# submarine0418/underwater_image_enhancement

Measured on AMD Instinct MI355X. Metric: megapixels/sec enhanced, higher is better.
Workload: dtype f32/f64

## Files before the change

### underwater_image_enhancement_amd/csrc/k_fused.hip

```cpp
#include <cstdlib>

#include "common.h"
#include "devutil.h"
#include "restore.h"

namespace uwie {

namespace {


typedef float f32x2 __attribute__((ext_vector_type(2)));
#ifndef UWIE_CLAHE_PREFETCH
#define UWIE_CLAHE_PREFETCH 0
#endif
#ifndef UWIE_STRETCH_WAVES
#define UWIE_STRETCH_WAVES 5
#endif
#define UWIE_DESCALE(x, n) (((x) + (1 << ((n)-1))) >> (n))

template <bool LIN, bool COLLECT, int NW = 2, typename V = float>
__global__ void __launch_bounds__(256) k_restore_planar_hist(RestoreSrc S, int npx, V *__restrict__ planar,
                                                             uint32_t *__restrict__ ghist, LinState *__restrict__ lin,
                                                             V *__restrict__ lists, uint32_t cap)
{
// ... 357 lines not shown
    const RankWave X{img, tpl, ftab, a0, a1, a2, s_wlo, s_wspan, s_lo, s_hi, s_below, myq, wstg[wv],
                     &lin[3 * b].gcount[0], (uint32_t)(sizeof(LinState) / sizeof(uint32_t)),
                     lists + (size_t)(3 * b) * (kLinLists / kRankCapMul) * cap, cap, lane};

    const int step = gridDim.x * 1024, iters = (npx + step - 1) / step;
#define UWIE_RANK_LOAD4(p_, w_, tv_)                                                                                   \
    do {                                                                                                                \
        const u32_unaligned *q_ = reinterpret_cast<const u32_unaligned *>(img + (size_t)(p_) * 3);                      \
        (w_)[0] = q_[0]; (w_)[1] = q_[1]; (w_)[2] = q_[2];                                                              \
        const double2_a8 ta_ = *reinterpret_cast<const double2_a8 *>(tpl + (p_)),                                       \
                         tb_ = *reinterpret_cast<const double2_a8 *>(tpl + (p_) + 2);                                   \
        (tv_)[0] = ta_.x; (tv_)[1] = ta_.y; (tv_)[2] = tb_.x; (tv_)[3] = tb_.y;                                         \
    } while (0)
    uint32_t w_nx[3] = {0, 0, 0};
    double tv_nx[4] = {1.0, 1.0, 1.0, 1.0};
    bool have_nx = false;
    const int p_last = npx - 4;
    {
        const int p0 = (blockIdx.x * 256 + tid) * 4;
        have_nx = p0 + 4 <= npx;
        UWIE_RANK_LOAD4(min(p0, p_last), w_nx, tv_nx);
    }
    for (int it = 0; it < iters; ++it) {
        const int p = it * step + (blockIdx.x * 256 + tid) * 4;
        const bool have = have_nx;
        const uint32_t w0 = w_nx[0], w1 = w_nx[1], w2 = w_nx[2];
        const double tv[4] = {tv_nx[0], tv_nx[1], tv_nx[2], tv_nx[3]};
        {
            const int pn = p + step;
            have_nx = it + 1 < iters && pn + 4 <= npx;
            UWIE_RANK_LOAD4(min(pn, p_last), w_nx, tv_nx);
        }
        uint32_t fm = 0;
        seen += 4u * (uint32_t)__popcll(__ballot(have));
        if (have) {
            float y[4];
#pragma unroll
            for (int i = 0; i < 4; ++i) y[i] = __builtin_amdgcn_rcpf((float)tv[i]);
            const uint32_t ub[3][4] = {{w0 & 255, w0 >> 24, (w1 >> 16) & 255, (w2 >> 8) & 255},
                                       {(w0 >> 8) & 255, w1 & 255, w1 >> 24, (w2 >> 16) & 255},
                                       {(w0 >> 16) & 255, (w1 >> 8) & 255, w2 & 255, w2 >> 24}};
#pragma unroll
            for (int c = 0; c < 3; ++c) {
                const float ac = c == 0 ? a0 : c == 1 ? a1 : a2;
#pragma unroll
                for (int i = 0; i < 4; ++i) {
                    const float v = fmaf(ftab[c * 256 + (int)ub[c][i]], y[i], ac);
                    bool in = false;
#pragma unroll
                    for (int w = 0; w < NW; ++w) {
                        const bool ge = v >= elo[c * NW + w];
                        cnt[c * NW + w] += (uint32_t)__popcll(__ballot(ge));
                        in = in | (ge & (v <= ehi[c * NW + w]));
                    }
                    fm |= (uint32_t)in << (4 * c + i);
                }
                __builtin_amdgcn_sched_barrier(0);
            }
        }
        const bool ragged = !have && p < npx;
        const uint32_t nmine = (uint32_t)__popc(fm);
        if (__ballot(nmine != 0)) {
            uint32_t pre = 0, tot = 0;
#pragma unroll
            for (int bit = 0; bit < 4; ++bit) {
                const uint64_t mk = __ballot((nmine >> bit) & 1u);
                pre += (uint32_t)__popcll(mk & ((1ull << lane) - 1)) << bit;
                tot += (uint32_t)__popcll(mk) << bit;
            }
            uint32_t at = qn + pre;
            for (uint32_t f = fm; f; f &= f - 1, ++at) {
                const int k = __ffs(f) - 1;
                myq[at] = ((uint32_t)(p + (k & 3)) << 2) | (uint32_t)(k >> 2);
            }
            qn += tot;
            while (qn >= 64u) {
                qn -= 64u;
                rank_exact_batch(X, qn, 64u, true, sc);
            }
        }
        if (__ballot(ragged)) {
            const uint32_t n3 = ragged ? (uint32_t)(npx - p) * 3u : 0u;
            wave_lds_sync();
            if (ragged)
                for (uint32_t i = 0; i < n3; ++i) myq[qn + i] = ((uint32_t)(p + (int)(i / 3u)) << 2) | (i % 3u);
            const uint32_t m = (uint32_t)__builtin_amdgcn_readfirstlane((int)__shfl((int)n3, (int)__builtin_ctzll(__ballot(ragged))));
            rank_exact_batch(X, qn, m, false, sc);
        }
    }
    if (qn) rank_exact_batch(X, 0u, qn, true, sc);
#pragma unroll
    for (int j = 0; j < NS; ++j)
        if (sc[j]) rank_flush_stage(X, j, sc[j]);
#pragma unroll
    for (int j = 0; j < NS; ++j) {
        uint32_t k = cnt[j];
#pragma unroll
        for (int o = 32; o > 0; o >>= 1) k = max(k, (uint32_t)__shfl_xor((int)k, o));
        if (lane == 0 && seen != k) atomicAdd(&s_below[j], seen - k);
    }
    __syncthreads();
    if (tid < NS && s_below[tid]) atomicAdd(&lin[3 * b + tid / NW].below[tid % NW], s_below[tid]);
}

struct Stretch {
    StretchDiv d1[3], d2[3];
    float lo1[3], lo2[3];
    int two;
    __device__ __forceinline__ void load(const float *pct, int b, int stride, float eps, int two_)
    {
        two = two_;
#pragma unroll
        for (int c = 0; c < 3; ++c) {
            const float *p = pct + (size_t)(b * 3 + c) * stride;
            lo1[c] = p[0];
            d1[c].set((p[1] - p[0]) + eps);
            lo2[c] = two ? p[2] : 0.f;
            d2[c].set(two ? (p[3] - p[2]) + eps : 1.f);
        }
    }
    __device__ __forceinline__ float apply(float v, int c) const
    {
        v = clip01(d1[c].quot_unit(v - lo1[c]));
        if (two) v = clip01(d2[c].quot_unit(v - lo2[c]));
        return v;
    }
    __device__ __forceinline__ bool allfast() const { return !two && d1[0].fast && d1[1].fast && d1[2].fast; }
    __device__ __forceinline__ void codes4(const float (&v)[4], int c, uint32_t (&code)[4]) const
    {
        const float den = d1[c].den, y = d1[c].y, lo = lo1[c];
        const f32x2 nd = {-den, -den}, yy = {y, y};
#pragma unroll
        for (int h = 0; h < 2; ++h) {
            const f32x2 n = f32x2{v[2 * h], v[2 * h + 1]} - lo;
            f32x2 q = n * y;
            q = __builtin_elementwise_fma(__builtin_elementwise_fma(nd, q, n), yy, q);
            q = __builtin_elementwise_fma(__builtin_elementwise_fma(nd, q, n), yy, q);
            const f32x2 s = f32x2{clip01(q.x), clip01(q.y)} * 255.0f;
            code[2 * h] = (uint32_t)(int)s.x;
            code[2 * h + 1] = (uint32_t)(int)s.y;
        }
    }
    __device__ __forceinline__ float apply_exact(float v, int c) const
    {
        v = clip01(d1[c].quot(v - lo1[c]));
        if (two) v = clip01(d2[c].quot(v - lo2[c]));
        return v;
    }
};

struct ClaheGeom {
    int H, W, tx, ty, tw, th, clip;
    float lutScale;
};

template <int SRC, int BS = 256>
__global__ void __launch_bounds__(BS) __attribute__((amdgpu_waves_per_eu(BS == 256 ? UWIE_STRETCH_WAVES : 4, 8))) k_stretch_lab_lut(const LabTables *__restrict__ T, const float *__restrict__ planar,
                                                         RestoreSrc src, const float *__restrict__ pct, int pct_stride,
                                                         float eps, int two, const uint8_t *__restrict__ codes, ClaheGeom g,
                                                         uint8_t *__restrict__ lab, uint8_t *__restrict__ lut)
{
    __shared__ uint32_t h[4][256];
    __shared__ uint32_t wsum[4];
    __shared__ uint16_t s_gamma[256], s_cbrt[3072];
    __shared__ int s_fwd[9];
    const int tile = blockIdx.x, b = blockIdx.y, tid = threadIdx.x, w = (tid >> 6) & 3, w4 = w;
    for (int i = tid; i < 1024; i += BS) (&h[0][0])[i] = 0;
    for (int i = tid; i < 256; i += BS) s_gamma[i] = T->gamma[i];
    for (int i = tid; i < 3072; i += BS) s_cbrt[i] = T->cbrt[i];
    if (tid < 9) s_fwd[tid] = T->fwd[tid];
    __shared__ uint16_t s_gcode[SRC == 2 ? 768 : 1];
    Stretch S;
    if (SRC != 2) S.load(pct, b, pct_stride, eps, two);
    if (SRC == 2)
        for (int i = tid; i < 768; i += BS) s_gcode[i] = T->gamma[codes[(size_t)b * 768 + i]];
    __syncthreads();
    const int npx = g.H * g.W;
    const float *r0 = planar + (size_t)b * 3 * npx, *r1 = r0 + npx, *r2 = r1 + npx;
    const uint8_t *img8 = src.in + (size_t)b * npx * 3;
    __shared__ double dtab[SRC == 1 ? 768 : 1];
    auto pixels = [&](auto &R) {
    if (SRC == 1) {
        R.init(src, b, (size_t)npx, dtab);
        __syncthreads();
    }
    uint8_t *labimg = lab + (size_t)b * npx * 3;
    const int ty = tile / g.tx, txi = tile % g.tx;
    const int area = g.tw * g.th;
    constexpr int Lscale = (116 * 255 + 50) / 100;
    constexpr int Lshift = -((16 * 255 * (1 << 15) + 50) / 100);
    auto to_lab = [&](float v0, float v1, float v2, uint32_t &L, uint32_t &a, uint32_t &bb) {
        const int R = SRC == 2 ? s_gcode[(int)v0] : s_gamma[quant_u8(S.apply(v0, 0))];
        const int G = SRC == 2 ? s_gcode[256 + (int)v1] : s_gamma[quant_u8(S.apply(v1, 1))];
        const int B = SRC == 2 ? s_gcode[512 + (int)v2] : s_gamma[quant_u8(S.apply(v2, 2))];
        const int fX = s_cbrt[UWIE_DESCALE(R * s_fwd[0] + G * s_fwd[1] + B * s_fwd[2], 12)];
        const int fY = s_cbrt[UWIE_DESCALE(R * s_fwd[3] + G * s_fwd[4] + B * s_fwd[5], 12)];
        const int fZ = s_cbrt[UWIE_DESCALE(R * s_fwd[6] + G * s_fwd[7] + B * s_fwd[8], 12)];
        L = sat_u8(UWIE_DESCALE(Lscale * fY + Lshift, 15));
        a = sat_u8(UWIE_DESCALE(500 * (fX - fY) + 128 * (1 << 15), 15));
        bb = sat_u8(UWIE_DESCALE(200 * (fY - fZ) + 128 * (1 << 15), 15));
    };
    const int x_lo = txi * g.tw, x_hi = min(x_lo + g.tw, g.W), y_lo = ty * g.th, y_hi = min(y_lo + g.th, g.H);
    const int gpr = max((x_hi - x_lo + 3) / 4, 0), total = max(y_hi - y_lo, 0) * gpr;
    const uint32_t gmagic = (uint32_t)(((1ull << 32) + max(gpr, 1) - 1) / max(gpr, 1));
    const int f0 = T->fwd[0], f1 = T->fwd[1], f2 = T->fwd[2], f3 = T->fwd[3], f4 = T->fwd[4], f5 = T->fwd[5], f6 = T->fwd[6],
              f7 = T->fwd[7], f8 = T->fwd[8];
    auto lab_of = [&](uint32_t Rg, uint32_t Gg, uint32_t Bg, uint32_t &L, uint32_t &a, uint32_t &bb) {
        const uint32_t ix = (__umul24(Rg, f0) + __umul24(Gg, f1) + __umul24(Bg, f2) + 2048u) >> 12;
        const uint32_t iy = (__umul24(Rg, f3) + __umul24(Gg, f4) + __umul24(Bg, f5) + 2048u) >> 12;
        const uint32_t iz = (__umul24(Rg, f6) + __umul24(Gg, f7) + __umul24(Bg, f8) + 2048u) >> 12;
        const int fX = s_cbrt[ix], fY = s_cbrt[iy], fZ = s_cbrt[iz];
        auto sat15 = [](int x) { return (uint32_t)min(max(x, 0), (256 << 15) - 1) >> 15; };
        L = sat15(__mul24(Lscale, fY) + (Lshift + (1 << 14)));
        a = sat15(__mul24(500, fX - fY) + (128 * (1 << 15) + (1 << 14)));
        bb = sat15(__mul24(200, fY - fZ) + (128 * (1 << 15) + (1 << 14)));
    };
    const bool fastpath = SRC == 1 && S.allfast();
    auto group_at = [&](int gi, int &n, int &p) {
        const int row = gpr == 1 ? gi : (int)__umulhi((uint32_t)gi, gmagic), xg = gi - row * gpr;
        const int x0 = x_lo + 4 * xg;
        n = min(4, x_hi - x0);
        p = (y_lo + row) * g.W + x0;
    };
    uint32_t w_nx[3] = {0, 0, 0};
    double tv_nx[4] = {1.0, 1.0, 1.0, 1.0};
    bool have_nx = false;
    if (SRC == 1 && fastpath && tid < total) {
        int n0, p0;
        group_at(tid, n0, p0);
        have_nx = n0 == 4;
        if (have_nx) R.load_four(p0, w_nx, tv_nx);
    }
    for (int gi = tid; gi < total; gi += BS) {
        int n, p;
        group_at(gi, n, p);
        const bool have = have_nx;
        const uint32_t w[3] = {w_nx[0], w_nx[1], w_nx[2]};
        const double tv[4] = {tv_nx[0], tv_nx[1], tv_nx[2], tv_nx[3]};
        have_nx = false;
        if (SRC == 1 && fastpath && gi + BS < total) {
            int nn, pn;
            group_at(gi + BS, nn, pn);
            have_nx = nn == 4;
            if (have_nx) R.load_four(pn, w_nx, tv_nx);
        }
        if (SRC == 1 && have) {
            float v[3][4];
            R.four_raw(w, tv, v);
            uint32_t code[3][4];
#pragma unroll
            for (int c = 0; c < 3; ++c) {
                const float r[4] = {clip01(v[c][0]), clip01(v[c][1]), clip01(v[c][2]), clip01(v[c][3])};
                S.codes4(r, c, code[c]);
            }
            uint32_t L[4], a[4], bb[4];
#pragma unroll
            for (int i = 0; i < 4; ++i) lab_of(s_gamma[code[0][i]], s_gamma[code[1][i]], s_gamma[code[2][i]], L[i], a[i], bb[i]);
            uint32_t cl = L[0], cn = 1;
#pragma unroll
            for (int i = 1; i < 4; ++i) {
                if (L[i] == cl) {
                    ++cn;
                } else {
                    atomicAdd(&h[w4][cl], cn);
                    cl = L[i];
                    cn = 1;
                }
            }
            atomicAdd(&h[w4][cl], cn);
            u32_unaligned *wd = reinterpret_cast<u32_unaligned *>(labimg + (size_t)p * 3);
            wd[0] = L[0] | (a[0] << 8) | (bb[0] << 16) | (L[1] << 24);
            wd[1] = a[1] | (bb[1] << 8) | (L[2] << 16) | (a[2] << 24);
            wd[2] = bb[2] | (L[3] << 8) | (a[3] << 16) | (bb[3] << 24);
            continue;
        }
        float v0[4], v1[4], v2[4];
        if (SRC == 2) {
            const Px4 q = n == 4 ? load_px4_any(img8 + (size_t)p * 3) : load_px4(img8 + (size_t)p * 3, n, false);
#pragma unroll
            for (int i = 0; i < 4; ++i) {
                v0[i] = (float)q.r[i];
                v1[i] = (float)q.g[i];
                v2[i] = (float)q.b[i];
            }
        } else if (SRC == 1) {
            float r[3][4];
            R.four(p, n, r);
#pragma unroll
            for (int i = 0; i < 4; ++i) {
                v0[i] = r[0][i];
                v1[i] = r[1][i];
                v2[i] = r[2][i];
            }
        } else if (n == 4) {
            *reinterpret_cast<uint4 *>(v0) = *reinterpret_cast<const u128_unaligned *>(r0 + p);
            *reinterpret_cast<uint4 *>(v1) = *reinterpret_cast<const u128_unaligned *>(r1 + p);
            *reinterpret_cast<uint4 *>(v2) = *reinterpret_cast<const u128_unaligned *>(r2 + p);
        } else {
#pragma unroll
            for (int i = 0; i < 4; ++i) {
                v0[i] = i < n ? r0[p + i] : 0.f;
                v1[i] = i < n ? r1[p + i] : 0.f;
                v2[i] = i < n ? r2[p + i] : 0.f;
            }
        }
        uint32_t L[4], a[4], bb[4];
#pragma unroll
        for (int i = 0; i < 4; ++i) to_lab(v0[i], v1[i], v2[i], L[i], a[i], bb[i]);
        uint32_t cl = L[0], cn = 1;
#pragma unroll
        for (int i = 1; i < 4; ++i) {
            if (i >= n) break;
            if (L[i] == cl) {
                ++cn;
            } else {
                atomicAdd(&h[w4][cl], cn);
                cl = L[i];
                cn = 1;
            }
        }
        atomicAdd(&h[w4][cl], cn);
        uint8_t *o = labimg + (size_t)p * 3;
        if (n == 4) {
            u32_unaligned *wd = reinterpret_cast<u32_unaligned *>(o);
            wd[0] = L[0] | (a[0] << 8) | (bb[0] << 16) | (L[1] << 24);
            wd[1] = a[1] | (bb[1] << 8) | (L[2] << 16) | (a[2] << 24);
            wd[2] = bb[2] | (L[3] << 8) | (a[3] << 16) | (bb[3] << 24);
        } else {
            for (int i = 0; i < n; ++i) {
                o[3 * i] = (uint8_t)L[i];
                o[3 * i + 1] = (uint8_t)a[i];
                o[3 * i + 2] = (uint8_t)bb[i];
            }
        }
    }
    if (x_lo + g.tw > g.W || y_lo + g.th > g.H) {
        for (int i = tid; i < area; i += BS) {
            const int ey = ty * g.th + i / g.tw, ex = txi * g.tw + i % g.tw;
            if (ey < g.H && ex < g.W) continue;
            const int p = reflect101(ey, g.H) * g.W + reflect101(ex, g.W);
            uint32_t L, a, bb;
            float e0, e1, e2;
            if (SRC == 2) {
                e0 = (float)img8[(size_t)p * 3];
                e1 = (float)img8[(size_t)p * 3 + 1];
                e2 = (float)img8[(size_t)p * 3 + 2];
            } else if (SRC == 1) {
                R.pixel(p, e0, e1, e2);
            } else {
                e0 = r0[p];
                e1 = r1[p];
                e2 = r2[p];
            }
            to_lab(e0, e1, e2, L, a, bb);
            atomicAdd(&h[w][L], 1u);
        }
    }
    };
    if (SRC == 1 && src.t32) {
        RestoreImgT<2, true> R;
        pixels(R);
    } else {
        RestoreImgT<2> R;
        pixels(R);
    }
    __syncthreads();
    if (BS > 256 && tid >= 256) return;
    uint32_t c = h[0][tid] + h[1][tid] + h[2][tid] + h[3][tid];
    if (g.clip > 0) {
        const uint32_t over = c > (uint32_t)g.clip ? c - g.clip : 0;
        if (over) c = g.clip;
        const uint32_t tot = block_incl_scan_256(over, wsum);
        __syncthreads();
        if (tid == 255) wsum[0] = tot;
        __syncthreads();
        const uint32_t clipped = wsum[0];
        __syncthreads();
        const uint32_t batch = clipped / 256, residual = clipped - batch * 256;
        c += batch;
        if (residual) {
            const uint32_t step = max(256u / residual, 1u);
            if (tid % step == 0 && tid / step < residual) c += 1;
        }
    }
    const uint32_t sum = block_incl_scan_256(c, wsum);
    lut[((size_t)b * g.tx * g.ty + tile) * 256 + tid] = sat_u8(__float2int_rn((float)sum * g.lutScale));
}


__device__ __forceinline__ float final_value(int v, int gamma_mode, float gexp)
{
    float y = (float)v / 255.0f;
    if (gamma_mode == 1) y = pow_f32(y, gexp);
    else if (gamma_mode == 2) y = clip01(pow_f32(y, gexp));
    return y;
}

__device__ __forceinline__ int ab_to_xz(int i)
{
    const int t = __mul24(i, 108);
    const uint32_t tp = (uint32_t)(t + ((t >> 31) & 840) + 841 * 1100);
    const int lin = (int)__umulhi(tp, 5106980u) - (1100 + 290);
    const uint32_t sq = __umul24((uint32_t)i, (uint32_t)i) >> 14;
    const int cub = (int)(__umul24(sq, (uint32_t)i) >> 14);
    return i <= 3390 ? lin : cub;
}
__device__ __forceinline__ int ab_to_xz_cubic(int i)
{
    const uint32_t sq = __umul24((uint32_t)i, (uint32_t)i) >> 14;
    return (int)(__umul24(sq, (uint32_t)i) >> 14);
}

#define UWIE_APPLY_WALKS(gpr, rstep) ((gpr) <= 256 && (rstep) * (gpr) * 8 >= 256 * 7)
constexpr bool clahe_apply_walks(int gpr) { return UWIE_APPLY_WALKS(gpr, 256 / (gpr > 1 ? gpr : 1)); }
static_assert(clahe_apply_walks(1) && clahe_apply_walks(45) && clahe_apply_walks(85), "walk: narrow cells");
static_assert(!clahe_apply_walks(86) && !clahe_apply_walks(90) && !clahe_apply_walks(111), "flat: 341 .. 444 px");
static_assert(clahe_apply_walks(112) && clahe_apply_walks(128), "walk: 445 .. 512 px");
static_assert(!clahe_apply_walks(129) && !clahe_apply_walks(223), "flat: 513 .. 892 px");
static_assert(clahe_apply_walks(224) && clahe_apply_walks(256) && !clahe_apply_walks(257), "walk up to 1024 px, flat beyond");

template <bool CODES, bool F32OUT>
__global__ void __launch_bounds__(256) k_clahe_apply_out(const LabTables *__restrict__ T, const uint8_t *__restrict__ lab,
                                                         const uint8_t *__restrict__ lut, ClaheGeom g, int nchunk,
                                                         int gamma_mode, float gexp, const uint8_t *__restrict__ fin_code,
                                                         const float *__restrict__ fin_val, uint8_t *__restrict__ out_u8,
                                                         float *__restrict__ out_f32, uint8_t *__restrict__ codes_out,
                                                         uint32_t *__restrict__ hist)
{
    constexpr int NF = CODES ? 768 : 256;
    constexpr bool TWOSTEP = CODES || F32OUT;
    constexpr int BASE = 1 << 14;
    __shared__ __attribute__((aligned(16))) int s_l[256][4];
    __shared__ int s_l2[256];
    __shared__ uint8_t s_invgamma[TWOSTEP ? 4096 : 1];
    __shared__ uint8_t s_fin[TWOSTEP ? 1 : 4096];
    __shared__ float s_ff[NF];
    __shared__ uint8_t s_fu[NF];
    __shared__ uint32_t s_h[CODES ? 4 * 768 : 1];
    __shared__ uint32_t s_lut4[4][256];
    const int tid = threadIdx.x, b = blockIdx.y;
    const int cell = blockIdx.x / nchunk, chunk = blockIdx.x - cell * nchunk;
    const int cyi = cell / (g.tx + 1), cxi = cell - cyi * (g.tx + 1);
    const int cx0 = max(cxi * g.tw - g.tw / 2, 0), cx1 = min((cxi + 1) * g.tw - g.tw / 2, g.W);
    const int ry0 = max(cyi * g.th - g.th / 2, 0), ry1 = min((cyi + 1) * g.th - g.th / 2, g.H);
    const int rows_per = (ry1 - ry0 + nchunk - 1) / nchunk;
    const int cy0 = ry0 + chunk * rows_per, cy1 = min(cy0 + rows_per, ry1);
    if (cx0 >= cx1 || cy0 >= cy1) return;
    const int wx0 = min(max(cxi - 2, 0), max(g.tx - 4, 0)), wy0 = min(max(cyi - 2, 0), max(g.ty - 4, 0));
    const int m0 = T->inv[0], m1 = T->inv[1], m2 = T->inv[2], m3 = T->inv[3], m4 = T->inv[4], m5 = T->inv[5], m6 = T->inv[6],
              m7 = T->inv[7], m8 = T->inv[8];
    {
        const int yy = T->ltoyf[2 * tid], ify = T->ltoyf[2 * tid + 1];
        *reinterpret_cast<int4 *>(&s_l[tid][0]) = make_int4(ify - 128 * BASE / 500, ify + (128 * BASE / 200 - 1), m1 * yy + (1 << 13), m4 * yy + (1 << 13));
        s_l2[tid] = m7 * yy + (1 << 13);
    }
    if (TWOSTEP)
        for (int i = tid; i < 4096; i += 256) s_invgamma[i] = T->invgamma[i];
    if (CODES) {
        for (int i = tid; i < 768; i += 256) {
            s_fu[i] = fin_code ? fin_code[(size_t)b * 768 + i] : (uint8_t)0;
            s_ff[i] = fin_val ? fin_val[(size_t)b * 768 + i] : 0.f;
        }
        if (hist)
            for (int i = tid; i < 4 * 768; i += 256) s_h[i] = 0;
    } else {
        const float y = final_value(tid, gamma_mode, gexp);
        s_ff[tid] = y;
        s_fu[tid] = (uint8_t)quant_u8(y);
    }
    const uint8_t *Lt = lut + (size_t)b * g.tx * g.ty * 256;
    {
        const int wy = tid >> 6, q = tid & 63;
        const int tyy = min(wy0 + wy, g.ty - 1);
        uint32_t d[4];
#pragma unroll
        for (int wx = 0; wx < 4; ++wx)
            d[wx] = reinterpret_cast<const uint32_t *>(Lt + (size_t)(tyy * g.tx + min(wx0 + wx, g.tx - 1)) * 256)[q];
#pragma unroll
        for (int k = 0; k < 4; ++k)
            s_lut4[wy][4 * q + k] = ((d[0] >> (8 * k)) & 255u) | (((d[1] >> (8 * k)) & 255u) << 8) | (((d[2] >> (8 * k)) & 255u) << 16) |
                                    (((d[3] >> (8 * k)) & 255u) << 24);
    }
    __syncthreads();
    if (!TWOSTEP) {
        for (int i = tid; i < 1024; i += 256) {
            const uint32_t q = reinterpret_cast<const uint32_t *>(T->invgamma)[i];
            reinterpret_cast<uint32_t *>(s_fin)[i] = (uint32_t)s_fu[q & 255] | ((uint32_t)s_fu[(q >> 8) & 255] << 8) |
                                                     ((uint32_t)s_fu[(q >> 16) & 255] << 16) | ((uint32_t)s_fu[q >> 24] << 24);
        }
        __syncthreads();
    }
    const float inv_tw = 1.0f / (float)g.tw, inv_th = 1.0f / (float)g.th;
    const int gpr = (cx1 - cx0 + 3) / 4, total = (cy1 - cy0) * gpr;
    const uint32_t gmagic = (uint32_t)(((1ull << 32) + gpr - 1) / gpr);
    struct Cols {
        uint32_t sel[4];
        float xa[4], xa1[4];
    };
    auto cols_of = [&](int x0) {
        Cols C;
#pragma unroll
        for (int i = 0; i < 4; ++i) {
            const int x = min(x0 + i, g.W - 1);
            const float txf = (float)x * inv_tw - 0.5f;
            int tx1 = (int)floorf(txf);
            int tx2 = tx1 + 1;
            C.xa[i] = txf - (float)tx1;
            C.xa1[i] = 1.0f - C.xa[i];
            tx1 = max(tx1, 0);
            tx2 = min(tx2, g.tx - 1);
            const uint32_t c1 = (uint32_t)min(max(tx1 - wx0, 0), 3), c2 = (uint32_t)min(max(tx2 - wx0, 0), 3);
            C.sel[i] = c1 | ((4u + c1) << 8) | (c2 << 16) | ((4u + c2) << 24);
        }
        return C;
    };
    auto fetch = [&](int row, int xg, uint32_t (&w)[3]) {
        const int y = cy0 + row, x0 = cx0 + 4 * xg;
        if (row < cy1 - cy0 && x0 + 4 <= cx1) {
            const u32_unaligned *q = reinterpret_cast<const u32_unaligned *>(lab + (((size_t)b * g.H + y) * g.W + x0) * 3);
            w[0] = q[0]; w[1] = q[1]; w[2] = q[2];
        }
    };
    auto group = [&](int row, int xg, const Cols &C, const uint32_t (&pre)[3], bool has_pre) {
        const int y = cy0 + row, x0 = cx0 + 4 * xg, n = min(4, cx1 - x0);
        const size_t pix = ((size_t)b * g.H + y) * g.W + x0;
        Px4 in4;
        if (n == 4) {
            uint32_t w0 = pre[0], w1 = pre[1], w2 = pre[2];
            if (!has_pre) {
                const u32_unaligned *w = reinterpret_cast<const u32_unaligned *>(lab + pix * 3);
                w0 = w[0]; w1 = w[1]; w2 = w[2];
            }
            in4.r[0] = w0 & 255; in4.g[0] = (w0 >> 8) & 255; in4.b[0] = (w0 >> 16) & 255;
            in4.r[1] = w0 >> 24; in4.g[1] = w1 & 255; in4.b[1] = (w1 >> 8) & 255;
            in4.r[2] = (w1 >> 16) & 255; in4.g[2] = w1 >> 24; in4.b[2] = w2 & 255;
            in4.r[3] = (w2 >> 8) & 255; in4.g[3] = (w2 >> 16) & 255; in4.b[3] = w2 >> 24;
        } else {
            in4 = load_px4(lab + pix * 3, n, false);
        }
        const float tyf = (float)y * inv_th - 0.5f;
        int ty1 = (int)floorf(tyf);
        int ty2 = ty1 + 1;
        const float ya = tyf - (float)ty1, ya1 = 1.0f - ya;
        ty1 = max(ty1, 0);
        ty2 = min(ty2, g.ty - 1);
        const uint32_t *row1 = s_lut4[min(max(ty1 - wy0, 0), 3)], *row2 = s_lut4[min(max(ty2 - wy0, 0), 3)];
        const f32x2 yw = {ya1, ya};
        uint32_t o0[4], o1[4], o2[4];
        int ix[4], iz[4], yt0[4], yt1[4], yt2[4];
#pragma unroll
        for (int i = 0; i < 4; ++i) {
            const int v = in4.r[i], aa = in4.g[i], bb = in4.b[i];
            const uint32_t pk = __builtin_amdgcn_perm(row2[v], row1[v], C.sel[i]);
            const f32x2 l1 = {(float)(pk & 255u), (float)((pk >> 8) & 255u)};
            const f32x2 l2 = {(float)((pk >> 16) & 255u), (float)(pk >> 24)};
            const f32x2 rw = (l1 * C.xa1[i] + l2 * C.xa[i]) * yw;
            const float res = rw.x + rw.y;
            const int LL = min(max(__float2int_rn(res), 0), 255);
            const int4 ly = *reinterpret_cast<const int4 *>(&s_l[LL][0]);
            yt0[i] = ly.z;
            yt1[i] = ly.w;
            yt2[i] = s_l2[LL];
            ix[i] = ly.x + (int)(((uint32_t)__umul24(aa, 5 * 53687) + (1u << 7)) >> 13);
            iz[i] = ly.y - (int)(((uint32_t)__umul24(bb, 41943) + (1u << 4)) >> 9);
        }
        int xx[4], zz[4];
        if (min(min(min(ix[0], ix[1]), min(ix[2], ix[3])), min(min(iz[0], iz[1]), min(iz[2], iz[3]))) > 3390) {
#pragma unroll
            for (int i = 0; i < 4; ++i) {
                xx[i] = ab_to_xz_cubic(ix[i]);
                zz[i] = ab_to_xz_cubic(iz[i]);
            }
// ... 459 lines not shown
```

### underwater_image_enhancement_amd/csrc/restore.h

```cpp
#pragma once
#include "common.h"
#include "devutil.h"

namespace uwie {

typedef double2 __attribute__((aligned(8))) double2_a8;

template <int TAB, bool F32 = false>
struct RestoreImgT {
    static constexpr bool t32 = F32;
    const uint8_t *img;
    const double *t;
    const float *tab;
    float a[3];
    bool att[3];
    __device__ __forceinline__ void init(const RestoreSrc &S, int b, size_t npx, void *lds_tab_v = nullptr)
    {
        float *lds_tab = static_cast<float *>(lds_tab_v);
        tab = lds_tab;
        const int k = S.kind ? S.kind[b] : 0;
        img = S.in + (size_t)b * npx * 3;
        t = F32 ? reinterpret_cast<const double *>(reinterpret_cast<const float *>(S.t) + (size_t)b * npx) : S.t + (size_t)b * npx;
#pragma unroll
        for (int c = 0; c < 3; ++c) {
            a[c] = S.A[b * 3 + c];
            att[c] = px_atten(k, c);
        }
        if (TAB) {
            for (int i = threadIdx.x; i < 768; i += blockDim.x) {
                const int c = i >> 8;
                const float x = px_norm_fast((uint32_t)(i & 255));
                const float d = ((c == 0 ? att[0] : c == 1 ? att[1] : att[2]) ? x * 0.85f : x) - (c == 0 ? a[0] : c == 1 ? a[1] : a[2]);
                if (TAB == 2 && !t32) static_cast<double *>(lds_tab_v)[i] = (double)d;
                else lds_tab[i] = d;
            }
        }
    }
    __device__ __forceinline__ double diff64(uint32_t u, int c) const
    {
        if (TAB == 2 && !t32) return reinterpret_cast<const double *>(tab)[c * 256 + u];
        return (double)diff(u, c);
    }
    __device__ __forceinline__ float diff(uint32_t u, int c) const
    {
        if (TAB == 2 && !t32) return (float)reinterpret_cast<const double *>(tab)[c * 256 + u];
        if (TAB) return tab[c * 256 + u];
        const float x = px_norm_fast(u);
        return (att[c] ? x * 0.85f : x) - a[c];
    }
    __device__ __forceinline__ float one(uint32_t u, int c, double tv) const
    {
        const float v = (float)((double)diff(u, c) / tv + (double)a[c]);
        return fminf(fmaxf(v, 0.0f), 1.0f);
    }
    __device__ __forceinline__ static bool recip_ok(double tv) { return tv >= 0x1p-100 && tv <= 0x1p100; }
    __device__ __forceinline__ static double recip(double tv)
    {
        double y = __builtin_amdgcn_rcp(tv);
        y = fma(y, fma(-tv, y, 1.0), y);
        return fma(y, fma(-tv, y, 1.0), y);
    }
    __device__ __forceinline__ float one_fast(uint32_t u, int c, double tv, double y) const
    {
        const double n = diff64(u, c), q0 = n * y;
        const float v = (float)(fma(fma(-tv, q0, n), y, q0) + (double)a[c]);
        return fminf(fmaxf(v, 0.0f), 1.0f);
    }
    __device__ __forceinline__ const float *tf() const { return reinterpret_cast<const float *>(t); }
    __device__ __forceinline__ static float recip32(float tv)
    {
        const float y = __builtin_amdgcn_rcpf(tv);
        return fmaf(fmaf(-tv, y, 1.0f), y, y);
    }
    __device__ __forceinline__ float one32_raw(uint32_t u, int c, float y) const { return fmaf(diff(u, c), y, a[c]); }
    __device__ __forceinline__ void pixel32(int p, float &r0, float &r1, float &r2) const
    {
        const uint8_t *q = img + (size_t)p * 3;
        const float y = recip32(tf()[p]);
        r0 = fminf(fmaxf(one32_raw(q[0], 0, y), 0.0f), 1.0f);
        r1 = fminf(fmaxf(one32_raw(q[1], 1, y), 0.0f), 1.0f);
        r2 = fminf(fmaxf(one32_raw(q[2], 2, y), 0.0f), 1.0f);
    }
    __device__ __forceinline__ float one_fast_raw(uint32_t u, int c, double tv, double y) const
    {
        const double n = diff64(u, c), q0 = n * y;
        return (float)(fma(fma(-tv, q0, n), y, q0) + (double)a[c]);
    }
    __device__ __forceinline__ void four_raw(const uint32_t (&w)[3], const double (&tv)[4], float (&r)[3][4]) const
    {
        const uint32_t w0 = w[0], w1 = w[1], w2 = w[2];
        const uint32_t ur[4] = {w0 & 255, w0 >> 24, (w1 >> 16) & 255, (w2 >> 8) & 255};
        const uint32_t ug[4] = {(w0 >> 8) & 255, w1 & 255, w1 >> 24, (w2 >> 16) & 255};
        const uint32_t ub[4] = {(w0 >> 16) & 255, (w1 >> 8) & 255, w2 & 255, w2 >> 24};
        if constexpr (F32) {
            typedef float f2 __attribute__((ext_vector_type(2)));
            float y[4];
#pragma unroll
            for (int i = 0; i < 4; ++i) y[i] = recip32(__int_as_float(__double2loint(tv[i])));
#pragma unroll
            for (int h = 0; h < 2; ++h) {
                const f2 yy = {y[2 * h], y[2 * h + 1]};
                const f2 r0 = __builtin_elementwise_fma(f2{diff(ur[2 * h], 0), diff(ur[2 * h + 1], 0)}, yy, f2{a[0], a[0]});
                const f2 r1 = __builtin_elementwise_fma(f2{diff(ug[2 * h], 1), diff(ug[2 * h + 1], 1)}, yy, f2{a[1], a[1]});
                const f2 r2 = __builtin_elementwise_fma(f2{diff(ub[2 * h], 2), diff(ub[2 * h + 1], 2)}, yy, f2{a[2], a[2]});
                r[0][2 * h] = r0.x; r[0][2 * h + 1] = r0.y;
                r[1][2 * h] = r1.x; r[1][2 * h + 1] = r1.y;
                r[2][2 * h] = r2.x; r[2][2 * h + 1] = r2.y;
            }
            return;
        }
#pragma unroll
        for (int i = 0; i < 4; ++i) {
            const double y = recip(tv[i]);
            r[0][i] = one_fast_raw(ur[i], 0, tv[i], y);
            r[1][i] = one_fast_raw(ug[i], 1, tv[i], y);
            r[2][i] = one_fast_raw(ub[i], 2, tv[i], y);
        }
    }
    __device__ __forceinline__ void load_four(int p, uint32_t (&w)[3], double (&tv)[4]) const
    {
        const u32_unaligned *q = reinterpret_cast<const u32_unaligned *>(img + (size_t)p * 3);
        w[0] = q[0]; w[1] = q[1]; w[2] = q[2];
        if constexpr (F32) {
            typedef float4 __attribute__((aligned(4))) float4_a4;
            const float4_a4 f = *reinterpret_cast<const float4_a4 *>(tf() + p);
            tv[0] = __hiloint2double(0, __float_as_int(f.x));
            tv[1] = __hiloint2double(0, __float_as_int(f.y));
            tv[2] = __hiloint2double(0, __float_as_int(f.z));
            tv[3] = __hiloint2double(0, __float_as_int(f.w));
            return;
        }
        const double2_a8 ta = *reinterpret_cast<const double2_a8 *>(t + p), tb = *reinterpret_cast<const double2_a8 *>(t + p + 2);
        tv[0] = ta.x; tv[1] = ta.y; tv[2] = tb.x; tv[3] = tb.y;
    }
    __device__ __forceinline__ void four(int p, int n, float (&r)[3][4]) const
    {
        if constexpr (F32) {
#pragma unroll
            for (int i = 0; i < 4; ++i) {
                r[0][i] = r[1][i] = r[2][i] = 0.0f;
                if (i < n) pixel32(p + i, r[0][i], r[1][i], r[2][i]);
            }
            return;
        }
        Px4 v;
        double tv[4];
        if (n == 4) {
            const u32_unaligned *w = reinterpret_cast<const u32_unaligned *>(img + (size_t)p * 3);
            const uint32_t w0 = w[0], w1 = w[1], w2 = w[2];
            v.r[0] = w0 & 255; v.g[0] = (w0 >> 8) & 255; v.b[0] = (w0 >> 16) & 255;
            v.r[1] = w0 >> 24; v.g[1] = w1 & 255; v.b[1] = (w1 >> 8) & 255;
            v.r[2] = (w1 >> 16) & 255; v.g[2] = w1 >> 24; v.b[2] = w2 & 255;
            v.r[3] = (w2 >> 8) & 255; v.g[3] = (w2 >> 16) & 255; v.b[3] = w2 >> 24;
            const double2_a8 ta = *reinterpret_cast<const double2_a8 *>(t + p), tb = *reinterpret_cast<const double2_a8 *>(t + p + 2);
            tv[0] = ta.x; tv[1] = ta.y; tv[2] = tb.x; tv[3] = tb.y;
        } else {
            v = load_px4(img + (size_t)p * 3, n, false);
#pragma unroll
            for (int i = 0; i < 4; ++i) tv[i] = i < n ? t[p + i] : 1.0;
        }
        if (recip_ok(tv[0]) && recip_ok(tv[1]) && recip_ok(tv[2]) && recip_ok(tv[3])) {
#pragma unroll
            for (int i = 0; i < 4; ++i) {
                const double y = recip(tv[i]);
                r[0][i] = one_fast(v.r[i], 0, tv[i], y);
                r[1][i] = one_fast(v.g[i], 1, tv[i], y);
                r[2][i] = one_fast(v.b[i], 2, tv[i], y);
            }
        } else {
#pragma unroll
            for (int i = 0; i < 4; ++i) {
                r[0][i] = one(v.r[i], 0, tv[i]);
                r[1][i] = one(v.g[i], 1, tv[i]);
                r[2][i] = one(v.b[i], 2, tv[i]);
            }
        }
    }
    __device__ __forceinline__ void pixel(int p, float &r0, float &r1, float &r2) const
    {
        if constexpr (F32) {
            pixel32(p, r0, r1, r2);
            return;
        }
        const uint8_t *q = img + (size_t)p * 3;
        const double tv = t[p];
        if (recip_ok(tv)) {
            const double y = recip(tv);
            r0 = one_fast(q[0], 0, tv, y);
            r1 = one_fast(q[1], 1, tv, y);
            r2 = one_fast(q[2], 2, tv, y);
        } else {
            r0 = one(q[0], 0, tv);
            r1 = one(q[1], 1, tv);
            r2 = one(q[2], 2, tv);
        }
    }
    __device__ __forceinline__ double one64(uint32_t u, int c, double tv) const
    {
        return fmin(fmax((double)diff(u, c) / tv + (double)a[c], 0.0), 1.0);
    }
    __device__ __forceinline__ double one64_fast(uint32_t u, int c, double tv, double y) const
    {
        const double n = (double)diff(u, c), q0 = n * y;
        return fmin(fmax(fma(fma(-tv, q0, n), y, q0) + (double)a[c], 0.0), 1.0);
    }
    __device__ __forceinline__ void four64(int p, int n, double (&r)[3][4]) const
    {
        Px4 v;
        double tv[4];
        if (n == 4) {
            v = load_px4_any(img + (size_t)p * 3);
            const double2_a8 ta = *reinterpret_cast<const double2_a8 *>(t + p), tb = *reinterpret_cast<const double2_a8 *>(t + p + 2);
            tv[0] = ta.x; tv[1] = ta.y; tv[2] = tb.x; tv[3] = tb.y;
        } else {
            v = load_px4(img + (size_t)p * 3, n, false);
#pragma unroll
            for (int i = 0; i < 4; ++i) tv[i] = i < n ? t[p + i] : 1.0;
        }
        if (recip_ok(tv[0]) && recip_ok(tv[1]) && recip_ok(tv[2]) && recip_ok(tv[3])) {
#pragma unroll
            for (int i = 0; i < 4; ++i) {
                const double y = recip(tv[i]);
                r[0][i] = one64_fast(v.r[i], 0, tv[i], y);
                r[1][i] = one64_fast(v.g[i], 1, tv[i], y);
                r[2][i] = one64_fast(v.b[i], 2, tv[i], y);
            }
        } else {
#pragma unroll
            for (int i = 0; i < 4; ++i) {
                r[0][i] = one64(v.r[i], 0, tv[i]);
                r[1][i] = one64(v.g[i], 1, tv[i]);
                r[2][i] = one64(v.b[i], 2, tv[i]);
            }
        }
    }
};

using RestoreImg = RestoreImgT<0>;
using RestoreImg32 = RestoreImgT<0, true>;

}
```

Measured before the change: 60180.

## Restructure stretch-LAB loop with incremental cursor, 32-bit addressing and double-buffered prefetch

Replaces the per-iteration magic-number division that mapped a group index to row/column in k_stretch_lab_lut with an incremental cursor that steps through the tile. Full 4-pixel groups go through a dedicated loop, unrolled by two, that ping-pongs prefetch buffers and uses 32-bit byte offsets (guarded by npx < 2^29). Narrow tiles can use a row 'walk' mode where each thread keeps a fixed column. Partial groups go through a separate slow loop. The aim is fewer integer address instructions and better load latency hiding, at the cost of more code complexity and some idle threads in walk mode.

Measured after the change: 60170. About the same (-0.0%).

```diff
diff --git a/profiles/stretch_loop_isa.py b/profiles/stretch_loop_isa.py
--- /dev/null
+++ b/profiles/stretch_loop_isa.py
@@ -0,0 +1,105 @@
+#!/usr/bin/env python3
+import re
+import sys
+
+import isa_summary as I
+
+KEY = "k_stretch_lab_lutILi1ELi256"
+
+
+def kernel_lines(path):
+    out, on = [], False
+    for line in open(path):
+        s = line.rstrip("\n")
+        if re.match(r"^_Z\w+:", s):
+            on = KEY in s
+        if on:
+            out.append(s)
+            if s.strip().startswith("s_endpgm"):
+                break
+    return out
+
+
+def meta(path):
+    m, on = {}, False
+    for line in open(path):
+        s = line.strip()
+        if s.startswith(".name:"):
+            on = KEY in s
+        elif on and re.match(r"^\.(vgpr_count|sgpr_count|vgpr_spill_count|sgpr_spill_count|private_segment_fixed_size):", s):
+            k, v = s.split(":")
+            m[k.strip(".")] = int(v)
+    return m
+
+
+def ops(lines):
+    return [t for t in (s.strip() for s in lines) if t and not t.startswith((";", ".", "//")) and not re.match(r"^\.?\w+:", t)]
+
+
+def loops(L):
+    pos = {m.group(1): i for i, s in enumerate(L) for m in [re.match(r"^(\.LBB\d+_\d+):", s.strip())] if m}
+    res = []
+    for i, s in enumerate(L):
+        p = s.split()
+        if p and p[0].startswith(("s_cbranch", "s_branch")) and len(p) > 1 and p[1] in pos and pos[p[1]] < i:
+            res.append((pos[p[1]], i))
+    return res
+
+
+def report(label, path, ranges):
+    L = kernel_lines(path)
+    print(f"## {label}: {meta(path)}")
+    if ranges:
+        body = [o for a, b in ranges for o in ops(L[a - 1:b])]
+        trips = 1
+        print(f"   blocks of the straight-line path, lines {ranges} of the kernel's listing (one trip)")
+    else:
+        cand = [l for l in loops(L) if sum(o.startswith("v_rcp_f64") for o in ops(L[l[0]:l[1] + 1])) >= 8
+                and not any(o.startswith("v_div_scale_f64") for o in ops(L[l[0]:l[1] + 1]))]
+        a, b = min(cand, key=lambda l: l[1] - l[0])
+        body = ops(L[a:b + 1])
+        trips = 2
+        print(f"   loop at lines {a + 1} - {b + 1} of the kernel's listing (two trips)")
+    n = lambda f: sum(1 for o in body if f(o.split()[0]))
+    mix = {}
+    for o in body:
+        k = I.classify(o.split()[0])
+        mix[k] = mix.get(k, 0) + 1
+    print(f"   {len(body)} instructions, {len(body) / trips:.0f} per trip: {I.fmt_mix(mix)}")
+    print("   v_mov*: %d  v_mul_lo_u32: %d  v_mul_hi_u32: %d  v_mad_u64_u32/v_mad_i64_i32: %d  v_lshl_add_u64: %d  s_waitcnt vmcnt: %d  "
+          "scratch_*: %d  v_readlane/v_writelane: %d" % (
+              n(lambda o: o.startswith("v_mov")), n(lambda o: o == "v_mul_lo_u32"), n(lambda o: o == "v_mul_hi_u32"),
+              n(lambda o: o.startswith(("v_mad_u64", "v_mad_i64"))), n(lambda o: o == "v_lshl_add_u64"),
+              sum(1 for o in body if o.startswith("s_waitcnt") and "vmcnt" in o), n(lambda o: o.startswith("scratch_")),
+              n(lambda o: o.startswith(("v_readlane", "v_writelane")))))
+    i = 0
+    while i < len(body):
+        if body[i].startswith("global_load_dwordx"):
+            j = i
+            while j + 1 < len(body) and any(b.startswith("global_load_dwordx") for b in body[j + 1:j + 4]):
+                j += 1
+            k = j + 1
+            while k < len(body) and not (body[k].startswith("s_waitcnt") and "vmcnt" in body[k]):
+                k += 1
+            dist = f"{k - j - 1} instructions later: {body[k]}" if k < len(body) else f"not in the rest of the listing ({len(body) - j - 1} instructions)"
+            print(f"   prefetch loads ({sum(b.startswith('global_load') for b in body[i:j + 1])}) at instruction {i}: first s_waitcnt vmcnt {dist}")
+            i = j + 1
+        else:
+            i += 1
+
+
+def main():
+    for a in sys.argv[1:]:
+        if a == "--list":
+            continue
+        label, _, rest = a.partition("=")
+        path, _, rg = rest.partition("@")
+        if "--list" in sys.argv:
+            for i, s in enumerate(kernel_lines(path), 1):
+                print(i, s)
+            continue
+        report(label, path, [tuple(int(x) for x in r.split("-")) for r in rg.split(",")] if rg else None)
+
+
+if __name__ == "__main__":
+    main()
diff --git a/underwater_image_enhancement_amd/csrc/k_fused.hip b/underwater_image_enhancement_amd/csrc/k_fused.hip
--- a/underwater_image_enhancement_amd/csrc/k_fused.hip
+++ b/underwater_image_enhancement_amd/csrc/k_fused.hip
@@ -533,6 +533,51 @@
 struct ClaheGeom {
     int H, W, tx, ty, tw, th, clip;
     float lutScale;
+};
+
+#define UWIE_APPLY_WALKS(gpr, rstep) ((gpr) <= 256 && (rstep) * (gpr) * 8 >= 256 * 7)
+constexpr bool clahe_apply_walks(int gpr) { return UWIE_APPLY_WALKS(gpr, 256 / (gpr > 1 ? gpr : 1)); }
+static_assert(clahe_apply_walks(1) && clahe_apply_walks(45) && clahe_apply_walks(85), "walk: narrow cells");
+static_assert(!clahe_apply_walks(86) && !clahe_apply_walks(90) && !clahe_apply_walks(111), "flat: 341 .. 444 px");
+static_assert(clahe_apply_walks(112) && clahe_apply_walks(128), "walk: 445 .. 512 px");
+static_assert(!clahe_apply_walks(129) && !clahe_apply_walks(223), "flat: 513 .. 892 px");
+static_assert(clahe_apply_walks(224) && clahe_apply_walks(256) && !clahe_apply_walks(257), "walk up to 1024 px, flat beyond");
+
+#ifndef UWIE_STRETCH_WALK
+#define UWIE_STRETCH_WALK 1
+#endif
+struct GroupSteps {
+    int ncols, dq, dr;
+    uint32_t step, wrap;
+    __device__ __forceinline__ GroupSteps(int ncols_, int BS, int W, bool walk = false)
+    {
+        ncols = ncols_;
+        dq = BS / ncols;
+        dr = walk ? 0 : BS - dq * ncols;
+        step = (uint32_t)(dq * W + 4 * dr);
+        wrap = (uint32_t)(W - 4 * ncols);
+    }
+};
+struct GroupCursor {
+    int row, xg;
+    uint32_t p;
+    __device__ __forceinline__ GroupCursor(int tid, const GroupSteps &G, uint32_t p00, int W)
+    {
+        row = tid / G.ncols;
+        xg = tid - row * G.ncols;
+        p = p00 + (uint32_t)(row * W + 4 * xg);
+    }
+    __device__ __forceinline__ void advance(const GroupSteps &G)
+    {
+        xg += G.dr;
+        row += G.dq;
+        p += G.step;
+        if ((!UWIE_STRETCH_WALK || G.dr) && xg >= G.ncols) {
+            xg -= G.ncols;
+            ++row;
+            p += G.wrap;
+        }
+    }
 };
 
 template <int SRC, int BS = 256>
@@ -582,8 +627,7 @@
         bb = sat_u8(UWIE_DESCALE(200 * (fY - fZ) + 128 * (1 << 15), 15));
     };
     const int x_lo = txi * g.tw, x_hi = min(x_lo + g.tw, g.W), y_lo = ty * g.th, y_hi = min(y_lo + g.th, g.H);
-    const int gpr = max((x_hi - x_lo + 3) / 4, 0), total = max(y_hi - y_lo, 0) * gpr;
-    const uint32_t gmagic = (uint32_t)(((1ull << 32) + max(gpr, 1) - 1) / max(gpr, 1));
+    const int gpr = max((x_hi - x_lo + 3) / 4, 0);
     const int f0 = T->fwd[0], f1 = T->fwd[1], f2 = T->fwd[2], f3 = T->fwd[3], f4 = T->fwd[4], f5 = T->fwd[5], f6 = T->fwd[6],
               f7 = T->fwd[7], f8 = T->fwd[8];
     auto lab_of = [&](uint32_t Rg, uint32_t Gg, uint32_t Bg, uint32_t &L, uint32_t &a, uint32_t &bb) {
@@ -596,65 +640,65 @@
         a = sat15(__mul24(500, fX - fY) + (128 * (1 << 15) + (1 << 14)));
         bb = sat15(__mul24(200, fY - fZ) + (128 * (1 << 15) + (1 << 14)));
     };
-    const bool fastpath = SRC == 1 && S.allfast();
-    auto group_at = [&](int gi, int &n, int &p) {
-        const int row = gpr == 1 ? gi : (int)__umulhi((uint32_t)gi, gmagic), xg = gi - row * gpr;
-        const int x0 = x_lo + 4 * xg;
-        n = min(4, x_hi - x0);
-        p = (y_lo + row) * g.W + x0;
-    };
-    uint32_t w_nx[3] = {0, 0, 0};
-    double tv_nx[4] = {1.0, 1.0, 1.0, 1.0};
-    bool have_nx = false;
-    if (SRC == 1 && fastpath && tid < total) {
-        int n0, p0;
-        group_at(tid, n0, p0);
-        have_nx = n0 == 4;
-        if (have_nx) R.load_four(p0, w_nx, tv_nx);
-    }
-    for (int gi = tid; gi < total; gi += BS) {
-        int n, p;
-        group_at(gi, n, p);
-        const bool have = have_nx;
-        const uint32_t w[3] = {w_nx[0], w_nx[1], w_nx[2]};
-        const double tv[4] = {tv_nx[0], tv_nx[1], tv_nx[2], tv_nx[3]};
-        have_nx = false;
-        if (SRC == 1 && fastpath && gi + BS < total) {
-            int nn, pn;
-            group_at(gi + BS, nn, pn);
-            have_nx = nn == 4;
-            if (have_nx) R.load_four(pn, w_nx, tv_nx);
-        }
-        if (SRC == 1 && have) {
-            float v[3][4];
-            R.four_raw(w, tv, v);
-            uint32_t code[3][4];
-#pragma unroll
-            for (int c = 0; c < 3; ++c) {
-                const float r[4] = {clip01(v[c][0]), clip01(v[c][1]), clip01(v[c][2]), clip01(v[c][3])};
-                S.codes4(r, c, code[c]);
-            }
-            uint32_t L[4], a[4], bb[4];
-#pragma unroll
-            for (int i = 0; i < 4; ++i) lab_of(s_gamma[code[0][i]], s_gamma[code[1][i]], s_gamma[code[2][i]], L[i], a[i], bb[i]);
-            uint32_t cl = L[0], cn = 1;
-#pragma unroll
-            for (int i = 1; i < 4; ++i) {
-                if (L[i] == cl) {
-                    ++cn;
-                } else {
-                    atomicAdd(&h[w4][cl], cn);
-                    cl = L[i];
-                    cn = 1;
+    const int nrows = max(y_hi - y_lo, 0);
+    const uint32_t p00 = (uint32_t)(y_lo * g.W + x_lo);
+    const bool fastpath = SRC == 1 && S.allfast() && npx < (1 << 29);
+    const int gfast = fastpath ? max(x_hi - x_lo, 0) / 4 : 0;
+    if (SRC == 1 && gfast > 0 && nrows > 0) {
+        const bool walks =UWIE_STRETCH_WALK && BS == 256 && UWIE_APPLY_WALKS(gfast, 256 / gfast);
+        const GroupSteps gs(gfast, BS, g.W, walks);
+        GroupCursor cur(tid, gs, p00, g.W);
+        if (walks && tid >= gs.dq * gfast) cur.row = nrows;
+        if (cur.row >= nrows) cur.p = p00;
+        auto trip = [&](const uint32_t (&wc)[3], const double (&tc)[4], uint32_t (&wn)[3], double (&tn)[4]) {
+            const bool have = cur.row < nrows;
+            const uint32_t p = cur.p;
+            cur.advance(gs);
+            if (cur.row >= nrows) cur.p = p;
+            R.load_four_at(cur.p, wn, tn);
+            if (have) {
+                float v[3][4];
+                R.four_raw(wc, tc, v);
+                uint32_t code[3][4];
+#pragma unroll
+                for (int c = 0; c < 3; ++c) {
+                    const float r[4] = {clip01(v[c][0]), clip01(v[c][1]), clip01(v[c][2]), clip01(v[c][3])};
+                    S.codes4(r, c, code[c]);
                 }
-            }
-            atomicAdd(&h[w4][cl], cn);
-            u32_unaligned *wd = reinterpret_cast<u32_unaligned *>(labimg + (size_t)p * 3);
-            wd[0] = L[0] | (a[0] << 8) | (bb[0] << 16) | (L[1] << 24);
-            wd[1] = a[1] | (bb[1] << 8) | (L[2] << 16) | (a[2] << 24);
-            wd[2] = bb[2] | (L[3] << 8) | (a[3] << 16) | (bb[3] << 24);
-            continue;
-        }
+                uint32_t L[4], a[4], bb[4];
+#pragma unroll
+                for (int i = 0; i < 4; ++i) lab_of(s_gamma[code[0][i]], s_gamma[code[1][i]], s_gamma[code[2][i]], L[i], a[i], bb[i]);
+                uint32_t cl = L[0], cn = 1;
+#pragma unroll
+                for (int i = 1; i < 4; ++i) {
+                    if (L[i] == cl) {
+                        ++cn;
+                    } else {
+                        atomicAdd(&h[w4][cl], cn);
+                        cl = L[i];
+                        cn = 1;
+                    }
+                }
+                atomicAdd(&h[w4][cl], cn);
+                u32_unaligned *wd = reinterpret_cast<u32_unaligned *>(labimg + p * 3u);
+                wd[0] = L[0] | (a[0] << 8) | (bb[0] << 16) | (L[1] << 24);
+                wd[1] = a[1] | (bb[1] << 8) | (L[2] << 16) | (a[2] << 24);
+                wd[2] = bb[2] | (L[3] << 8) | (a[3] << 16) | (bb[3] << 24);
+            }
+        };
+        uint32_t wa[3], wb[3];
+        double ta[4], tb[4];
+        R.load_four_at(cur.p, wa, ta);
+        const int trips = walks ? (nrows + gs.dq - 1) / gs.dq : (nrows * gfast + BS - 1) / BS;
+        for (int it = 0; it < trips; it += 2) {
+            trip(wa, ta, wb, tb);
+            trip(wb, tb, wa, ta);
+        }
+    }
+    const int gslow = gpr - gfast;
+    const GroupSteps gs(max(gslow, 1), BS, g.W);
+    for (GroupCursor cur(tid, gs, p00 + 4u * (uint32_t)gfast, g.W); gslow > 0 && cur.row < nrows; cur.advance(gs)) {
+        const int n = min(4, x_hi - (x_lo + 4 * (gfast + cur.xg))), p = (int)cur.p;
         float v0[4], v1[4], v2[4];
         if (SRC == 2) {
             const Px4 q = n == 4 ? load_px4_any(img8 + (size_t)p * 3) : load_px4(img8 + (size_t)p * 3, n, false);
@@ -791,14 +835,6 @@
     const uint32_t sq = __umul24((uint32_t)i, (uint32_t)i) >> 14;
     return (int)(__umul24(sq, (uint32_t)i) >> 14);
 }
-
-#define UWIE_APPLY_WALKS(gpr, rstep) ((gpr) <= 256 && (rstep) * (gpr) * 8 >= 256 * 7)
-constexpr bool clahe_apply_walks(int gpr) { return UWIE_APPLY_WALKS(gpr, 256 / (gpr > 1 ? gpr : 1)); }
-static_assert(clahe_apply_walks(1) && clahe_apply_walks(45) && clahe_apply_walks(85), "walk: narrow cells");
-static_assert(!clahe_apply_walks(86) && !clahe_apply_walks(90) && !clahe_apply_walks(111), "flat: 341 .. 444 px");
-static_assert(clahe_apply_walks(112) && clahe_apply_walks(128), "walk: 445 .. 512 px");
-static_assert(!clahe_apply_walks(129) && !clahe_apply_walks(223), "flat: 513 .. 892 px");
-static_assert(clahe_apply_walks(224) && clahe_apply_walks(256) && !clahe_apply_walks(257), "walk up to 1024 px, flat beyond");
 
 template <bool CODES, bool F32OUT>
 __global__ void __launch_bounds__(256) k_clahe_apply_out(const LabTables *__restrict__ T, const uint8_t *__restrict__ lab,
diff --git a/underwater_image_enhancement_amd/csrc/restore.h b/underwater_image_enhancement_amd/csrc/restore.h
--- a/underwater_image_enhancement_amd/csrc/restore.h
+++ b/underwater_image_enhancement_amd/csrc/restore.h
@@ -132,6 +132,24 @@
         }
         const double2_a8 ta = *reinterpret_cast<const double2_a8 *>(t + p), tb = *reinterpret_cast<const double2_a8 *>(t + p + 2);
         tv[0] = ta.x; tv[1] = ta.y; tv[2] = tb.x; tv[3] = tb.y;
+    }
+    __device__ __forceinline__ void load_four_at(uint32_t p, uint32_t (&w)[3], double (&tv)[4]) const
+    {
+        const u32_unaligned *q = reinterpret_cast<const u32_unaligned *>(img + p * 3u);
+        w[0] = q[0]; w[1] = q[1]; w[2] = q[2];
+        const char *tb = reinterpret_cast<const char *>(t);
+        if constexpr (F32) {
+            typedef float4 __attribute__((aligned(4))) float4_a4;
+            const float4_a4 f = *reinterpret_cast<const float4_a4 *>(tb + p * 4u);
+            tv[0] = __hiloint2double(0, __float_as_int(f.x));
+            tv[1] = __hiloint2double(0, __float_as_int(f.y));
+            tv[2] = __hiloint2double(0, __float_as_int(f.z));
+            tv[3] = __hiloint2double(0, __float_as_int(f.w));
+            return;
+        }
+        const double2_a8 *tp = reinterpret_cast<const double2_a8 *>(tb + p * 8u);
+        const double2_a8 ta = tp[0], tc = tp[1];
+        tv[0] = ta.x; tv[1] = ta.y; tv[2] = tc.x; tv[3] = tc.y;
     }
     __device__ __forceinline__ void four(int p, int n, float (&r)[3][4]) const
     {
```
